# yuxiaoxiangyong/Multilateral-Temporal-view-Pyramid-Transformer-for-Video-Inpainting-Detection

Hardware: AMD Instinct MI355X
Metric: clips/sec fwd (B=8,T=5,224x224) (higher is better)
Workload: dtype f32; 1 GPU; full Mumpy forward (3 temporal views, pyramid decoder), B=8 clips/GPU, T=5, 224x224, fp32, tubelets (5,4,1); global_batch=8, launch=hipGraph replay, fork/join over HIP streams (independent branches co-scheduled), parallelism=batch-sharded x1, one metric all-reduce

## Files before the change

multilateral-temporal-view-pyramid-transformer-for-video-inpainting-detection_amd/csrc/common.h:

```cpp
#pragma once
#include <hip/hip_runtime.h>
#include <stdint.h>
#include <stdio.h>
#include "../../include/mumpy_hip.h"

namespace mumpy {

typedef float f32x4 __attribute__((ext_vector_type(4)));
typedef float f32x16 __attribute__((ext_vector_type(16)));

constexpr int WAVE = 64;
constexpr int WS = 7;
constexpr int WT = 49;
constexpr int HD = 32;

void set_error(const char* fmt, ...);

#ifdef MUMPY_TUNING
int tune_int(const char* name, int dflt);
const char* tune_str(const char* name);
#else
inline int tune_int(const char*, int dflt) { return dflt; }
inline const char* tune_str(const char*) { return nullptr; }
#endif

inline hipStream_t as_stream(void* s) { return reinterpret_cast<hipStream_t>(s); }
inline bool aligned16(const void* p) { return (reinterpret_cast<uintptr_t>(p) & 15u) == 0; }

#define MUMPY_CHECK_LAUNCH(name)                                                     \
    do {                                                                             \
        hipError_t e_ = hipGetLastError();                                           \
        if (e_ != hipSuccess) {                                                      \
            mumpy::set_error("%s: launch failed: %s", name, hipGetErrorString(e_));  \
            return (int)e_;                                                          \
        }                                                                            \
    } while (0)

#define MUMPY_REQUIRE(cond, code, ...)                                               \
    do {                                                                             \
        if (!(cond)) {                                                               \
            mumpy::set_error(__VA_ARGS__);                                           \
            return code;                                                             \
        }                                                                            \
    } while (0)

__device__ __forceinline__ unsigned xcd_major_id(unsigned orig, unsigned nwg) {
    const unsigned xcd = orig & 7, q8 = nwg >> 3, r8 = nwg & 7;
    return (xcd < r8 ? xcd * (q8 + 1) : r8 * (q8 + 1) + (xcd - r8) * q8) + (orig >> 3);
}

template <int CTRL>
__device__ __forceinline__ float dpp_f(float v) {
    return __builtin_bit_cast(float, __builtin_amdgcn_update_dpp(0, __builtin_bit_cast(int, v), CTRL, 0xF, 0xF, true));
}
__device__ __forceinline__ float swz_xor16(float v) {
    return __builtin_bit_cast(float, __builtin_amdgcn_ds_swizzle(__builtin_bit_cast(int, v), (16 << 10) | 0x1f));
}

__device__ __forceinline__ float wave_sum(float v, int width) {
    if (width > 1) v += dpp_f<0xB1>(v);
    if (width > 2) v += dpp_f<0x4E>(v);
    if (width > 4) v += dpp_f<0x141>(v);
    if (width > 8) v += dpp_f<0x140>(v);
    if (width > 16) v += swz_xor16(v);
    if (width > 32) v += __shfl_xor(v, 32);
    return v;
}

template <typename T>
__device__ __forceinline__ T ordered_sum(T first, const T* __restrict__ p, int64_t stride, int n_more) {
    T s = first;
    int z = 0;
    for (; z + 8 <= n_more; z += 8) {
        T v[8];
#pragma unroll
        for (int u = 0; u < 8; ++u) v[u] = p[(int64_t)(z + u) * stride];
#pragma unroll
        for (int u = 0; u < 8; ++u) s += v[u];
    }
    for (; z < n_more; ++z) s += p[(int64_t)z * stride];
    return s;
}

__device__ __forceinline__ void gn_block_stats(const float* __restrict__ stats, int nsplit, int G, int b, double n, float eps,
                                               float* gm, float* gr, double (*red)[2]) {
    const int tid = threadIdx.x, nslice = 256 / G, g = tid % G, k = tid / G;
    double s = 0.0, q = 0.0;
    if (k < nslice)
        for (int sp = k; sp < nsplit; sp += nslice) {
            const float* o = stats + (((int64_t)b * nsplit + sp) * G + g) * 2;
            s += (double)o[0]; q += (double)o[1];
        }
    red[tid][0] = s; red[tid][1] = q;
    __syncthreads();
    if (tid < G) {
        double ss = 0.0, qq = 0.0;
        for (int j = 0; j < nslice; ++j) { ss += red[j * G + tid][0]; qq += red[j * G + tid][1]; }
        const double m = ss / n;
        double var = qq / n - m * m;
        if (var < 0.0) var = 0.0;
        gm[tid] = (float)m;
        gr[tid] = (float)(1.0 / sqrt(var + (double)eps));
    }
    __syncthreads();
}

__device__ __forceinline__ float erf_fast(float x) {
    const float ax = fabsf(x);
    const float t = __builtin_amdgcn_rcpf(fmaf(0.3275911f, ax, 1.0f));
    float p = fmaf(1.061405429f, t, -1.453152027f);
    p = fmaf(p, t, 1.421413741f);
    p = fmaf(p, t, -0.284496736f);
    p = fmaf(p, t, 0.254829592f);
    const float y = 1.0f - p * t * __expf(-ax * ax);
    return copysignf(y, x);
}

__device__ __forceinline__ float gelu_erf(float x) { return 0.5f * x * (1.0f + erf_fast(x * 0.70710678118654752440f)); }

__device__ __forceinline__ int window_token(int wy, int wx, int p, int Hs, int W, int shift) {
    int py = p / WS, px = p - py * WS;
    int y = wy * WS + py + shift;
    int x = wx * WS + px + shift;
    if (y >= Hs) y -= Hs;
    if (x >= W) x -= W;
    return y * W + x;
}

}
```

multilateral-temporal-view-pyramid-transformer-for-video-inpainting-detection_amd/csrc/cva_fused.hip:

```cpp
#include "common.h"
using namespace mumpy;

namespace {

constexpr int BK = 32, LDR = 36;

__device__ __forceinline__ void divmod49(unsigned m, unsigned& q, unsigned& r) {
    q = (unsigned)(((uint64_t)m * 2804876602ull) >> 37);
    r = m - 49u * q;
}

template <int C>
__global__ __launch_bounds__(256, 2) void deform_sample_kv_kernel(const float* __restrict__ x2, const float* __restrict__ pos,
                                                                  const float* __restrict__ Wkv, const float* __restrict__ bkv,
                                                                  float* __restrict__ kv, int Hs2, int W, int nWx, int nW2, int nq,
                                                                  int M, unsigned gn) {
    constexpr int BM = 64, BN = 192, TN = 3, N = 2 * C, K = C, CG = C / 3, NK = K / BK, CPG = CG / BK;
    constexpr int A_LD = BM / 32, B_LD = BN / 32;
    __shared__ __attribute__((aligned(16))) float lds[2][(BM + BN) * LDR];
    const int tid = threadIdx.x, lane = tid & 63, wave = tid >> 6;
    const int c = lane & 31, h = lane >> 5, wm = wave >> 1, wn = wave & 1;
    const unsigned wgid = xcd_major_id(blockIdx.x, gridDim.x);
    const unsigned tm = wgid / gn, tn = wgid - tm * gn;
    const int m0 = (int)tm * BM, n0 = (int)tn * BN;
    const int ld_row = tid >> 3, ld_c4 = tid & 7;

    const float* abase[A_LD];
    const float* apos[A_LD];
    int aoff[A_LD][4];
    float aw[A_LD][4];
#pragma unroll
    for (int i = 0; i < A_LD; ++i) {
        int m = m0 + ld_row + 32 * i;
        if (m > M - 1) m = M - 1;
        unsigned b2, p;
        divmod49((unsigned)m, b2, p);
        const unsigned b = b2 / (unsigned)nW2, n = b2 - b * (unsigned)nW2;
        const unsigned wy = n / (unsigned)nWx, wx = n - wy * (unsigned)nWx;
        abase[i] = x2 + (((int64_t)b * Hs2 + wy * WS) * W + wx * WS) * C + 4 * ld_c4;
        apos[i] = pos + ((int64_t)(b2 % (unsigned)nq) * 3 * WT + p) * 2;
    }
    auto set_group = [&](int g) {
#pragma unroll
        for (int i = 0; i < A_LD; ++i) {
            const float gy = apos[i][g * WT * 2], gx = apos[i][g * WT * 2 + 1];
            const float iy = ((gy + 1.0f) * 0.5f) * 6.0f;
            const float ix = ((gx + 1.0f) * 0.5f) * 6.0f;
            const float y0f = floorf(iy), x0f = floorf(ix);
            const int y0 = (int)y0f, x0 = (int)x0f;
            const float wgt[4] = {(x0f + 1.0f - ix) * (y0f + 1.0f - iy), (ix - x0f) * (y0f + 1.0f - iy),
                                  (x0f + 1.0f - ix) * (iy - y0f), (ix - x0f) * (iy - y0f)};
#pragma unroll
            for (int e = 0; e < 4; ++e) {
                const int yy = y0 + (e >> 1), xx = x0 + (e & 1);
                const bool ok = (unsigned)yy < (unsigned)WS && (unsigned)xx < (unsigned)WS;
                aw[i][e] = ok ? wgt[e] : 0.f;
                aoff[i][e] = ok ? (yy * W + xx) * C : 0;
            }
        }
    };
    const float* brow[B_LD];
#pragma unroll
    for (int i = 0; i < B_LD; ++i) {
        int n = n0 + ld_row + 32 * i;
        if (n > N - 1) n = N - 1;
        brow[i] = Wkv + (int64_t)n * K + 4 * ld_c4;
    }
    f32x4 areg[A_LD], breg[B_LD];
    auto gload = [&](int kc) {
        const int k0 = kc * BK;
#pragma unroll
        for (int i = 0; i < A_LD; ++i) {
            const float* s = abase[i] + k0;
            f32x4 r = *reinterpret_cast<const f32x4*>(s + aoff[i][0]) * aw[i][0];
            r += *reinterpret_cast<const f32x4*>(s + aoff[i][1]) * aw[i][1];
            r += *reinterpret_cast<const f32x4*>(s + aoff[i][2]) * aw[i][2];
            r += *reinterpret_cast<const f32x4*>(s + aoff[i][3]) * aw[i][3];
            areg[i] = r;
        }
#pragma unroll
        for (int i = 0; i < B_LD; ++i) breg[i] = *reinterpret_cast<const f32x4*>(brow[i] + k0);
    };
    auto lstore = [&](int buf) {
#pragma unroll
        for (int i = 0; i < A_LD; ++i) *reinterpret_cast<f32x4*>(&lds[buf][(ld_row + 32 * i) * LDR + 4 * ld_c4]) = areg[i];
#pragma unroll
        for (int i = 0; i < B_LD; ++i) *reinterpret_cast<f32x4*>(&lds[buf][(BM + ld_row + 32 * i) * LDR + 4 * ld_c4]) = breg[i];
    };
    f32x16 acc[TN];
#pragma unroll
    for (int j = 0; j < TN; ++j)
#pragma unroll
        for (int r = 0; r < 16; ++r) acc[j][r] = 0.f;
    auto compute = [&](int buf) {
        const float* a_f = &lds[buf][(wm * 32 + c) * LDR + 16 * h];
        const float* b_f = &lds[buf][(BM + wn * 96 + c) * LDR + 16 * h];
#pragma unroll
        for (int q = 0; q < 4; ++q) {
            const f32x4 fa = *reinterpret_cast<const f32x4*>(a_f + 4 * q);
            f32x4 fb[TN];
#pragma unroll
            for (int j = 0; j < TN; ++j) fb[j] = *reinterpret_cast<const f32x4*>(b_f + 32 * j * LDR + 4 * q);
#pragma unroll
            for (int e = 0; e < 4; ++e)
#pragma unroll
                for (int j = 0; j < TN; ++j) acc[j] = __builtin_amdgcn_mfma_f32_32x32x2f32(fa[e], fb[j][e], acc[j], 0, 0, 0);
        }
    };
    set_group(0);
    gload(0);
    lstore(0);
    __syncthreads();
    for (int kc = 0; kc < NK; ++kc) {
        if (kc + 1 < NK) {
            if ((kc + 1) % CPG == 0) set_group((kc + 1) / CPG);
            gload(kc + 1);
        }
        compute(kc & 1);
        if (kc + 1 < NK) lstore((kc + 1) & 1);
        __syncthreads();
    }
#pragma unroll
    for (int j = 0; j < TN; ++j) {
        const int n = n0 + wn * 96 + 32 * j + c;
        if (n >= N) continue;
        const float bv = bkv[n];
#pragma unroll
        for (int r = 0; r < 16; ++r) {
            const int m = m0 + wm * 32 + (r & 3) + 8 * (r >> 2) + 4 * h;
            if (m < M) kv[(int64_t)m * N + n] = acc[j][r] + bv;
        }
    }
}

template <int C>
__global__ __launch_bounds__(256, 2) void deform_out_combine_kernel(const float* __restrict__ o, const float* __restrict__ Wout,
                                                                   const float* __restrict__ bout, const float* __restrict__ x1,
                                                                   float* __restrict__ out, int H, int W, int nWx, int nWf, int MO,
                                                                   unsigned gn) {
    constexpr int BM = 64, BN = 64, K = C, NK = K / BK;
    constexpr int A_LD = BM / 32, B_LD = BN / 32;
    __shared__ __attribute__((aligned(16))) float lds[2][(BM + BN) * LDR];
    const int tid = threadIdx.x, lane = tid & 63, wave = tid >> 6;
    const int c = lane & 31, h = lane >> 5, wm = wave >> 1, wn = wave & 1;
    const unsigned wgid = xcd_major_id(blockIdx.x, gridDim.x);
    const unsigned tn = wgid / gn, tm = wgid - tn * gn;
    const int c0 = (int)tm * BM, m0 = (int)tn * BN;
    const int ld_row = tid >> 3, ld_c4 = tid & 7;
    const float* arow[A_LD];
    const float* brow[B_LD];
#pragma unroll
    for (int i = 0; i < A_LD; ++i) {
        int cc = c0 + ld_row + 32 * i;
        if (cc > C - 1) cc = C - 1;
        arow[i] = Wout + (int64_t)cc * K + 4 * ld_c4;
    }
#pragma unroll
    for (int i = 0; i < B_LD; ++i) {
        int m = m0 + ld_row + 32 * i;
        if (m > MO - 1) m = MO - 1;
        brow[i] = o + (int64_t)m * K + 4 * ld_c4;
    }
    f32x4 areg[A_LD], breg[B_LD];
    auto gload = [&](int kc) {
#pragma unroll
        for (int i = 0; i < A_LD; ++i) areg[i] = *reinterpret_cast<const f32x4*>(arow[i] + kc * BK);
#pragma unroll
        for (int i = 0; i < B_LD; ++i) breg[i] = *reinterpret_cast<const f32x4*>(brow[i] + kc * BK);
    };
    auto lstore = [&](int buf) {
#pragma unroll
        for (int i = 0; i < A_LD; ++i) *reinterpret_cast<f32x4*>(&lds[buf][(ld_row + 32 * i) * LDR + 4 * ld_c4]) = areg[i];
#pragma unroll
        for (int i = 0; i < B_LD; ++i) *reinterpret_cast<f32x4*>(&lds[buf][(BM + ld_row + 32 * i) * LDR + 4 * ld_c4]) = breg[i];
    };
    f32x16 acc;
#pragma unroll
    for (int r = 0; r < 16; ++r) acc[r] = 0.f;
    auto compute = [&](int buf) {
        const float* a_f = &lds[buf][(wm * 32 + c) * LDR + 16 * h];
        const float* b_f = &lds[buf][(BM + wn * 32 + c) * LDR + 16 * h];
#pragma unroll
        for (int q = 0; q < 4; ++q) {
            const f32x4 fa = *reinterpret_cast<const f32x4*>(a_f + 4 * q), fb = *reinterpret_cast<const f32x4*>(b_f + 4 * q);
#pragma unroll
            for (int e = 0; e < 4; ++e) acc = __builtin_amdgcn_mfma_f32_32x32x2f32(fa[e], fb[e], acc, 0, 0, 0);
        }
    };
    gload(0);
    lstore(0);
    __syncthreads();
    for (int kc = 0; kc < NK; ++kc) {
        if (kc + 1 < NK) gload(kc + 1);
        compute(kc & 1);
        if (kc + 1 < NK) lstore((kc + 1) & 1);
        __syncthreads();
    }
    const int m = m0 + wn * 32 + c;
    if (m >= MO) return;
    unsigned bw, pp;
    divmod49((unsigned)m, bw, pp);
    const unsigned b = bw / (unsigned)nWf, n = bw - b * (unsigned)nWf;
    const int wy = (int)(n / (unsigned)nWx), wx = (int)(n - (n / (unsigned)nWx) * (unsigned)nWx);
    const int64_t img = (int64_t)b * H * W;
    const int64_t win_base = (img + (int64_t)n * WT) * C;
#pragma unroll
    for (int r = 0; r < 16; ++r) {
        const int cc = c0 + wm * 32 + (r & 3) + 8 * (r >> 2) + 4 * h;
        if (cc >= C) continue;
        const int f = cc * WT + (int)pp;
        const int po = f / C, co = f - po * C;
        const int tok = window_token(wy, wx, po, H, W, 0);
        out[win_base + f] = x1[win_base + f] + x1[(img + tok) * C + co] + (acc[r] + bout[cc]);
    }
}

}

extern "C" int mumpy_deform_sample_kv_fwd(const float* x2, const float* pos, const float* Wkv, const float* bkv, float* kv, int B,
                                          int Hs2, int W, int C, int nq, void* stream) {
    MUMPY_REQUIRE(x2 && pos && Wkv && bkv && kv, MUMPY_ENULL, "deform_sample_kv: null pointer");
    MUMPY_REQUIRE(aligned16(x2) && aligned16(Wkv) && aligned16(kv), MUMPY_EALIGN, "deform_sample_kv: pointers must be 16-byte aligned");
    MUMPY_REQUIRE(B > 0 && Hs2 > 0 && W > 0 && Hs2 % WS == 0 && W % WS == 0 && nq > 0, MUMPY_EINVAL,
                  "deform_sample_kv: bad grid (%d,%d) / nq=%d", Hs2, W, nq);
    MUMPY_REQUIRE(C == 96 || C == 192 || C == 384 || C == 768, MUMPY_EINVAL,
                  "deform_sample_kv: C=%d is not one of the encoder widths 96/192/384/768", C);
    const int nWx = W / WS, nW2 = (Hs2 / WS) * nWx;
    const int64_t nwin = (int64_t)B * nW2, M = nwin * WT;
    MUMPY_REQUIRE(M < (1ll << 31) - 64, MUMPY_ERANGE, "deform_sample_kv: too many windows");
    const unsigned gn = (unsigned)((2 * C + 191) / 192);
    const int64_t grid = ((M + 63) / 64) * gn;
    MUMPY_REQUIRE(grid < (1ll << 31), MUMPY_ERANGE, "deform_sample_kv: too many tiles");
#define MUMPY_SKV(C_)                                                                                                     \
    hipLaunchKernelGGL(deform_sample_kv_kernel<C_>, dim3((unsigned)grid), dim3(256), 0, as_stream(stream), x2, pos, Wkv, bkv, \
                       kv, Hs2, W, nWx, nW2, nq, (int)M, gn)
    switch (C) {
        case 96: MUMPY_SKV(96); break;
        case 192: MUMPY_SKV(192); break;
        case 384: MUMPY_SKV(384); break;
        default: MUMPY_SKV(768); break;
    }
#undef MUMPY_SKV
    MUMPY_CHECK_LAUNCH("deform_sample_kv");
    return 0;
}

extern "C" int mumpy_deform_out_combine_fwd(const float* o, const float* Wout, const float* bout, const float* x1, float* out, int B,
                                            int H, int W, int C, void* stream) {
    MUMPY_REQUIRE(o && Wout && bout && x1 && out, MUMPY_ENULL, "deform_out_combine: null pointer");
    MUMPY_REQUIRE(x1 != out, MUMPY_EINVAL, "deform_out_combine: out must not alias x1");
    MUMPY_REQUIRE(aligned16(o) && aligned16(Wout), MUMPY_EALIGN, "deform_out_combine: pointers must be 16-byte aligned");
    MUMPY_REQUIRE(B > 0 && H > 0 && W > 0 && H % WS == 0 && W % WS == 0, MUMPY_EINVAL, "deform_out_combine: bad grid (%d,%d)", H, W);
    MUMPY_REQUIRE(C == 96 || C == 192 || C == 384 || C == 768, MUMPY_EINVAL,
                  "deform_out_combine: C=%d is not one of the encoder widths 96/192/384/768", C);
    const int nWx = W / WS, nWf = (H / WS) * nWx;
    const int64_t MO = (int64_t)B * nWf * WT;
    MUMPY_REQUIRE(MO * 49 < (1ll << 31) && MO < (1ll << 31) - 64, MUMPY_ERANGE, "deform_out_combine: too many windows");
    const unsigned gn = (unsigned)((C + 63) / 64);
    const int64_t grid = ((MO + 63) / 64) * gn;
#define MUMPY_OC(C_)                                                                                                      \
    hipLaunchKernelGGL(deform_out_combine_kernel<C_>, dim3((unsigned)grid), dim3(256), 0, as_stream(stream), o, Wout, bout, x1, \
                       out, H, W, nWx, nWf, (int)MO, gn)
    switch (C) {
        case 96: MUMPY_OC(96); break;
        case 192: MUMPY_OC(192); break;
        case 384: MUMPY_OC(384); break;
        default: MUMPY_OC(768); break;
    }
#undef MUMPY_OC
    MUMPY_CHECK_LAUNCH("deform_out_combine");
    return 0;
}
```

multilateral-temporal-view-pyramid-transformer-for-video-inpainting-detection_amd/csrc/deform.hip:

```cpp
#include <stdlib.h>
#include "common.h"
using namespace mumpy;

namespace {

template <int Cg>
__global__ __launch_bounds__(256) void deform_offsets_kernel(const float* __restrict__ q, const float* __restrict__ dw_w,
                                                             const float* __restrict__ dw_b,
                                                             const float* __restrict__ ln_g,
                                                             const float* __restrict__ ln_b,
                                                             const float* __restrict__ pw_w, float* __restrict__ pos,
                                                             int H, int W, int C, int nWx, int nWf) {
    constexpr int CP = Cg + 4;
    __shared__ __attribute__((aligned(16))) float sm[WT * Cg + WT * CP + 25 * Cg + 4 * Cg];
    float* tile = sm;
    float* conv = sm + WT * Cg;
    float* wsm = conv + WT * CP;
    float* par = wsm + 25 * Cg;
    const int bw = blockIdx.x, g = blockIdx.y;
    const int b = bw / nWf, n = bw - b * nWf;
    const int wy = n / nWx, wx = n - wy * nWx;
    const int tid = threadIdx.x;
    const int64_t L = (int64_t)H * W;
    const float* qb = q + (int64_t)b * L * C + g * Cg;
    const int cg4 = Cg >> 2;
    {
        constexpr int NT = WT * (Cg / 4), PT = (NT + 255) / 256;
        f32x4 v[PT];
#pragma unroll
        for (int u = 0; u < PT; ++u) {
            const int idx = tid + 256 * u;
            if (idx < NT) {
                const int p = idx / cg4, c4 = idx - p * cg4;
                v[u] = *reinterpret_cast<const f32x4*>(qb + (int64_t)window_token(wy, wx, p, H, W, 0) * C + 4 * c4);
            }
        }
#pragma unroll
        for (int u = 0; u < PT; ++u) {
            const int idx = tid + 256 * u;
            if (idx < NT) { const int p = idx / cg4, c4 = idx - p * cg4; *reinterpret_cast<f32x4*>(tile + p * Cg + 4 * c4) = v[u]; }
        }
        constexpr int NW = 25 * Cg / 4, PW = (NW + 255) / 256;
        f32x4 t[PW];
#pragma unroll
        for (int u = 0; u < PW; ++u) { const int idx = tid + 256 * u; if (idx < NW) t[u] = reinterpret_cast<const f32x4*>(dw_w)[idx]; }
#pragma unroll
        for (int u = 0; u < PW; ++u) { const int idx = tid + 256 * u; if (idx < NW) reinterpret_cast<f32x4*>(wsm)[idx] = t[u]; }
    }
    for (int idx = tid; idx < Cg; idx += 256) {
        par[idx] = ln_g[idx];
        par[Cg + idx] = ln_b[idx];
        par[2 * Cg + idx] = pw_w[idx];
        par[3 * Cg + idx] = pw_w[Cg + idx];
    }
    const int cc = tid % Cg;
    const float breg = dw_b[cc];
    __syncthreads();
    float wreg[25];
#pragma unroll
    for (int i = 0; i < 25; ++i) wreg[i] = wsm[cc * 25 + i];
    for (int p = tid / Cg; p < WT; p += 256 / Cg) {
        const int py = p / WS, px = p - py * WS;
        float acc = breg;
#pragma unroll
        for (int dy = 0; dy < 5; ++dy) {
            const int yy = py + dy - 2;
            const bool vy = (unsigned)yy < (unsigned)WS;
            const int yc = vy ? yy : py;
#pragma unroll
            for (int dx = 0; dx < 5; ++dx) {
                const int xx = px + dx - 2;
                const bool ok = vy && (unsigned)xx < (unsigned)WS;
                const int xc = ok ? xx : px;
                const float t = tile[(yc * WS + xc) * Cg + cc];
                acc = fmaf(ok ? t : 0.f, wreg[dy * 5 + dx], acc);
            }
        }
        conv[p * CP + cc] = acc;
    }
    __syncthreads();
    const int p = tid >> 2, qd = tid & 3;
    if (p < WT) {
        const float* cv = conv + p * CP;
        float s = 0.f;
#pragma unroll 8
        for (int ch = qd; ch < Cg; ch += 4) s += cv[ch];
        s += __shfl_xor(s, 1);
        s += __shfl_xor(s, 2);
        const float mean = s / (float)Cg;
        float qq = 0.f;
#pragma unroll 8
        for (int ch = qd; ch < Cg; ch += 4) { const float d = cv[ch] - mean; qq = fmaf(d, d, qq); }
        qq += __shfl_xor(qq, 1);
        qq += __shfl_xor(qq, 2);
        const float rstd = rsqrtf(qq / (float)Cg + 1e-5f);
        float oy = 0.f, ox = 0.f;
#pragma unroll 4
        for (int ch = qd; ch < Cg; ch += 4) {
            const float a = gelu_erf((cv[ch] - mean) * rstd * par[ch] + par[Cg + ch]);
            oy = fmaf(a, par[2 * Cg + ch], oy);
            ox = fmaf(a, par[3 * Cg + ch], ox);
        }
        oy += __shfl_xor(oy, 1);
        oy += __shfl_xor(oy, 2);
        ox += __shfl_xor(ox, 1);
        ox += __shfl_xor(ox, 2);
        if (qd == 0) {
            const int py = p / WS, px = p - py * WS;
            const float ry = ((0.5f + (float)py) / 7.0f) * 2.0f - 1.0f;
            const float rx = ((0.5f + (float)px) / 7.0f) * 2.0f - 1.0f;
            const float rng = 1.0f / 7.0f;
            float* o = pos + (((int64_t)bw * 3 + g) * WT + p) * 2;
            o[0] = tanhf(oy) * rng * 2.0f + ry;
            o[1] = tanhf(ox) * rng * 2.0f + rx;
        }
    }
}

template <int C>
__global__ __launch_bounds__(256) void deform_sample_kernel(const float* __restrict__ x2, const float* __restrict__ pos,
                                                            float* __restrict__ out, int Hs2, int W, int nWx, int nW2,
                                                            int nq) {
    constexpr int C4N = C / 4, CG = C / 3;
    const int b2 = blockIdx.x;
    const int b = b2 / nW2, n = b2 - b * nW2;
    const int wy = n / nWx, wx = n - wy * nWx;
    const float* base = x2 + ((int64_t)b * Hs2 * W + (int64_t)wy * WS * W + wx * WS) * C;
    const float* pw = pos + (int64_t)(b2 % nq) * 3 * WT * 2;
    float* ob = out + (int64_t)b2 * WT * C;
    for (int idx = threadIdx.x; idx < WT * C4N; idx += 256) {
        const int p = idx / C4N, c4 = idx - p * C4N;
        const int g = (4 * c4) / CG;
        const float gy = pw[(g * WT + p) * 2], gx = pw[(g * WT + p) * 2 + 1];
        const float iy = ((gy + 1.0f) * 0.5f) * 6.0f;
        const float ix = ((gx + 1.0f) * 0.5f) * 6.0f;
        const float y0f = floorf(iy), x0f = floorf(ix);
        const int y0 = (int)y0f, x0 = (int)x0f;
        const float wnw = (x0f + 1.0f - ix) * (y0f + 1.0f - iy);
        const float wne = (ix - x0f) * (y0f + 1.0f - iy);
        const float wsw = (x0f + 1.0f - ix) * (iy - y0f);
        const float wse = (ix - x0f) * (iy - y0f);
        const float* src = base + 4 * c4;
        auto corner = [&](int yy, int xx) -> f32x4 {
            if (yy < 0 || yy >= WS || xx < 0 || xx >= WS) return f32x4{0, 0, 0, 0};
            return *reinterpret_cast<const f32x4*>(src + (yy * W + xx) * C);
        };
        f32x4 r = corner(y0, x0) * wnw;
        r += corner(y0, x0 + 1) * wne;
        r += corner(y0 + 1, x0) * wsw;
        r += corner(y0 + 1, x0 + 1) * wse;
        *reinterpret_cast<f32x4*>(ob + idx * 4) = r;
    }
}

template <int C>
__global__ __launch_bounds__(256) void deform_sample_lds_kernel(const float* __restrict__ x2, const float* __restrict__ pos,
                                                                float* __restrict__ out, int Hs2, int W, int nWx, int nW2,
                                                                int nq) {
    constexpr int SL = 96, S4 = SL / 4, CG = C / 3;
    __shared__ __attribute__((aligned(16))) float tile[WT * SL];
    const int b2 = blockIdx.x, slab = blockIdx.y;
    const int b = b2 / nW2, n = b2 - b * nW2;
    const int wy = n / nWx, wx = n - wy * nWx;
    const float* base = x2 + ((int64_t)b * Hs2 * W + (int64_t)wy * WS * W + wx * WS) * C + slab * SL;
    for (int idx = threadIdx.x; idx < WT * S4; idx += 256) {
        const int tok = idx / S4, j = idx - tok * S4;
        const int ty = tok / WS, tx = tok - ty * WS;
        *reinterpret_cast<f32x4*>(&tile[tok * SL + 4 * j]) = *reinterpret_cast<const f32x4*>(base + (ty * W + tx) * C + 4 * j);
    }
    __syncthreads();
    const float* pw = pos + (int64_t)(b2 % nq) * 3 * WT * 2;
    float* ob = out + (int64_t)b2 * WT * C + slab * SL;
    for (int idx = threadIdx.x; idx < WT * S4; idx += 256) {
        const int p = idx / S4, c4 = idx - p * S4;
        const int g = (slab * SL + 4 * c4) / CG;
        const float gy = pw[(g * WT + p) * 2], gx = pw[(g * WT + p) * 2 + 1];
        const float iy = ((gy + 1.0f) * 0.5f) * 6.0f;
        const float ix = ((gx + 1.0f) * 0.5f) * 6.0f;
        const float y0f = floorf(iy), x0f = floorf(ix);
        const int y0 = (int)y0f, x0 = (int)x0f;
        const float wnw = (x0f + 1.0f - ix) * (y0f + 1.0f - iy);
        const float wne = (ix - x0f) * (y0f + 1.0f - iy);
        const float wsw = (x0f + 1.0f - ix) * (iy - y0f);
        const float wse = (ix - x0f) * (iy - y0f);
        auto corner = [&](int yy, int xx) -> f32x4 {
            if (yy < 0 || yy >= WS || xx < 0 || xx >= WS) return f32x4{0, 0, 0, 0};
            return *reinterpret_cast<const f32x4*>(&tile[(yy * WS + xx) * SL + 4 * c4]);
        };
        f32x4 r = corner(y0, x0) * wnw;
        r += corner(y0, x0 + 1) * wne;
        r += corner(y0 + 1, x0) * wsw;
        r += corner(y0 + 1, x0 + 1) * wse;
        *reinterpret_cast<f32x4*>(ob + p * C + 4 * c4) = r;
    }
}

__global__ __launch_bounds__(256) void deform_combine_kernel(const float* __restrict__ x1, const float* __restrict__ Yt,
                                                             float* __restrict__ out, int H, int W, int C, int nWx,
                                                             int nWf) {
    __shared__ float tile[WT * 33];
    const int bw = blockIdx.x, cb = blockIdx.y;
    const int b = bw / nWf, n = bw - b * nWf;
    const int wy = n / nWx, wx = n - wy * nWx;
    const int tid = threadIdx.x;
    const float* ys = Yt + (int64_t)bw * WT * C + cb * 32;
    for (int idx = tid; idx < WT * 32; idx += 256) {
        const int p = idx >> 5, cc = idx & 31;
        tile[p * 33 + cc] = ys[(int64_t)p * C + cc];
    }
    __syncthreads();
    const int64_t img = (int64_t)b * H * W;
    const int64_t win_base = (img + (int64_t)n * WT) * C;
    const int f0 = cb * 32 * WT;
    for (int idx = tid; idx < WT * 32; idx += 256) {
        const int f = f0 + idx;
        const int cl = idx / WT, pp = idx - cl * WT;
        const int po = f / C, co = f - po * C;
        const int tok = window_token(wy, wx, po, H, W, 0);
        out[win_base + f] = x1[win_base + f] + x1[(img + tok) * C + co] + tile[pp * 33 + cl];
    }
}

__global__ __launch_bounds__(256) void add_kernel(const float* __restrict__ a, const float* __restrict__ b,
                                                  float* __restrict__ o, int64_t n4) {
    for (int64_t i = (int64_t)blockIdx.x * 256 + threadIdx.x; i < n4; i += (int64_t)gridDim.x * 256)
        reinterpret_cast<f32x4*>(o)[i] = reinterpret_cast<const f32x4*>(a)[i] + reinterpret_cast<const f32x4*>(b)[i];
}

}

extern "C" int mumpy_deform_offsets_fwd(const float* q, const float* dw_w, const float* dw_b, const float* ln_g,
                                        const float* ln_b, const float* pw_w, float* pos, int B, int H, int W, int C,
                                        void* stream) {
    MUMPY_REQUIRE(q && dw_w && dw_b && ln_g && ln_b && pw_w && pos, MUMPY_ENULL, "deform_offsets: null pointer");
    MUMPY_REQUIRE(aligned16(q) && aligned16(dw_w), MUMPY_EALIGN, "deform_offsets: q and the depthwise weights must be 16-byte aligned");
    MUMPY_REQUIRE(B > 0 && H % WS == 0 && W % WS == 0 && H > 0 && W > 0, MUMPY_EINVAL, "deform_offsets: bad grid (%d,%d)", H, W);
    const int Cg = C / 3;
    MUMPY_REQUIRE(C % 3 == 0 && (Cg == 32 || Cg == 64 || Cg == 128 || Cg == 256), MUMPY_EINVAL,
                  "deform_offsets: group width C/3=%d must be 32, 64, 128 or 256", Cg);
    const int nWx = W / WS, nWf = (H / WS) * nWx;
#define MUMPY_OFFS(CG)                                                                                              \
    hipLaunchKernelGGL(deform_offsets_kernel<CG>, dim3(B * nWf, 3), dim3(256), 0, as_stream(stream), q, dw_w, dw_b, ln_g, \
                       ln_b, pw_w, pos, H, W, C, nWx, nWf)
    switch (Cg) {
        case 32: MUMPY_OFFS(32); break;
        case 64: MUMPY_OFFS(64); break;
        case 128: MUMPY_OFFS(128); break;
        default: MUMPY_OFFS(256); break;
    }
#undef MUMPY_OFFS
    MUMPY_CHECK_LAUNCH("deform_offsets");
    return 0;
}

extern "C" int mumpy_deform_sample_fwd(const float* x2, const float* pos, float* out, int B, int Hs2, int W, int C,
                                       int nq, void* stream) {
    MUMPY_REQUIRE(x2 && pos && out, MUMPY_ENULL, "deform_sample: null pointer");
    MUMPY_REQUIRE(aligned16(x2) && aligned16(out), MUMPY_EALIGN, "deform_sample: pointers must be 16-byte aligned");
    MUMPY_REQUIRE(B > 0 && Hs2 > 0 && W > 0 && Hs2 % WS == 0 && W % WS == 0 && nq > 0, MUMPY_EINVAL,
                  "deform_sample: bad grid (%d,%d) / nq=%d", Hs2, W, nq);
    MUMPY_REQUIRE(C == 96 || C == 192 || C == 384 || C == 768, MUMPY_EINVAL,
                  "deform_sample: C=%d is not one of the encoder widths 96/192/384/768", C);
    const int nWx = W / WS, nW2 = (Hs2 / WS) * nWx;
    const int64_t nwin = (int64_t)B * nW2;
    MUMPY_REQUIRE(nwin < (1ll << 31), MUMPY_ERANGE, "deform_sample: too many windows");
    static const bool direct = tune_int("MUMPY_SAMPLE_DIRECT", 0) != 0;
#define MUMPY_SAMPLE(C_)                                                                                             \
    if (direct)                                                                                                      \
        hipLaunchKernelGGL(deform_sample_kernel<C_>, dim3((unsigned)nwin), dim3(256), 0, as_stream(stream), x2, pos, out,  \
                           Hs2, W, nWx, nW2, nq);                                                                    \
    else                                                                                                             \
        hipLaunchKernelGGL(deform_sample_lds_kernel<C_>, dim3((unsigned)nwin, C_ / 96), dim3(256), 0, as_stream(stream), x2, \
                           pos, out, Hs2, W, nWx, nW2, nq)
    switch (C) {
        case 96: MUMPY_SAMPLE(96); break;
        case 192: MUMPY_SAMPLE(192); break;
        case 384: MUMPY_SAMPLE(384); break;
        default: MUMPY_SAMPLE(768); break;
    }
#undef MUMPY_SAMPLE
    MUMPY_CHECK_LAUNCH("deform_sample");
    return 0;
}

extern "C" int mumpy_deform_combine_fwd(const float* x1, const float* Yt, float* out, int B, int H, int W, int C,
                                        void* stream) {
    MUMPY_REQUIRE(x1 && Yt && out, MUMPY_ENULL, "deform_combine: null pointer");
    MUMPY_REQUIRE(x1 != out, MUMPY_EINVAL, "deform_combine: out must not alias x1");
    MUMPY_REQUIRE(B > 0 && H > 0 && W > 0 && H % WS == 0 && W % WS == 0 && C % 32 == 0, MUMPY_EINVAL,
                  "deform_combine: bad shape (%d,%d,%d)", H, W, C);
    const int nWx = W / WS, nWf = (H / WS) * nWx;
    hipLaunchKernelGGL(deform_combine_kernel, dim3(B * nWf, C / 32), dim3(256), 0, as_stream(stream), x1, Yt, out, H, W,
                       C, nWx, nWf);
    MUMPY_CHECK_LAUNCH("deform_combine");
    return 0;
}

extern "C" int mumpy_add_fwd(const float* a, const float* b, float* out, int64_t n, void* stream) {
    MUMPY_REQUIRE(a && b && out, MUMPY_ENULL, "add: null pointer");
    MUMPY_REQUIRE(aligned16(a) && aligned16(b) && aligned16(out) && n % 4 == 0 && n >= 0, MUMPY_EALIGN,
                  "add: need 16-byte aligned pointers and n %% 4 == 0");
    if (n == 0) return 0;
    int64_t grid = (n / 4 + 255) / 256;
    if (grid > 4096) grid = 4096;
    hipLaunchKernelGGL(add_kernel, dim3((unsigned)grid), dim3(256), 0, as_stream(stream), a, b, out, n / 4);
    MUMPY_CHECK_LAUNCH("add");
    return 0;
}
```

Baseline: 375.1 clips/s.

## Specialize deform kernels for small grids with deeper prefetch and row-split offsets

```diff
diff --git a/multilateral-temporal-view-pyramid-transformer-for-video-inpainting-detection_amd/csrc/common.h b/multilateral-temporal-view-pyramid-transformer-for-video-inpainting-detection_amd/csrc/common.h
--- a/multilateral-temporal-view-pyramid-transformer-for-video-inpainting-detection_amd/csrc/common.h
+++ b/multilateral-temporal-view-pyramid-transformer-for-video-inpainting-detection_amd/csrc/common.h
@@ -13,6 +13,7 @@
 constexpr int WS = 7;
 constexpr int WT = 49;
 constexpr int HD = 32;
+constexpr int CHIP_CUS = 256;
 
 void set_error(const char* fmt, ...);
 
diff --git a/multilateral-temporal-view-pyramid-transformer-for-video-inpainting-detection_amd/csrc/cva_fused.hip b/multilateral-temporal-view-pyramid-transformer-for-video-inpainting-detection_amd/csrc/cva_fused.hip
--- a/multilateral-temporal-view-pyramid-transformer-for-video-inpainting-detection_amd/csrc/cva_fused.hip
+++ b/multilateral-temporal-view-pyramid-transformer-for-video-inpainting-detection_amd/csrc/cva_fused.hip
@@ -10,7 +10,7 @@
     r = m - 49u * q;
 }
 
-template <int C>
+template <int C, bool AHEAD>
 __global__ __launch_bounds__(256, 2) void deform_sample_kv_kernel(const float* __restrict__ x2, const float* __restrict__ pos,
                                                                   const float* __restrict__ Wkv, const float* __restrict__ bkv,
                                                                   float* __restrict__ kv, int Hs2, int W, int nWx, int nW2, int nq,
@@ -26,7 +26,7 @@
     const int ld_row = tid >> 3, ld_c4 = tid & 7;
 
     const float* abase[A_LD];
-    const float* apos[A_LD];
+    float gpy[A_LD][3], gpx[A_LD][3];
     int aoff[A_LD][4];
     float aw[A_LD][4];
 #pragma unroll
@@ -38,12 +38,19 @@
         const unsigned b = b2 / (unsigned)nW2, n = b2 - b * (unsigned)nW2;
         const unsigned wy = n / (unsigned)nWx, wx = n - wy * (unsigned)nWx;
         abase[i] = x2 + (((int64_t)b * Hs2 + wy * WS) * W + wx * WS) * C + 4 * ld_c4;
-        apos[i] = pos + ((int64_t)(b2 % (unsigned)nq) * 3 * WT + p) * 2;
+        const float* ap = pos + ((int64_t)(b2 % (unsigned)nq) * 3 * WT + p) * 2;
+#pragma unroll
+        for (int g = 0; g < 3; ++g) {
+            const float2 gp = *reinterpret_cast<const float2*>(ap + g * WT * 2);
+            gpy[i][g] = gp.x;
+            gpx[i][g] = gp.y;
+        }
     }
     auto set_group = [&](int g) {
 #pragma unroll
         for (int i = 0; i < A_LD; ++i) {
-            const float gy = apos[i][g * WT * 2], gx = apos[i][g * WT * 2 + 1];
+            const float gy = g == 0 ? gpy[i][0] : g == 1 ? gpy[i][1] : gpy[i][2];
+            const float gx = g == 0 ? gpx[i][0] : g == 1 ? gpx[i][1] : gpx[i][2];
             const float iy = ((gy + 1.0f) * 0.5f) * 6.0f;
             const float ix = ((gx + 1.0f) * 0.5f) * 6.0f;
             const float y0f = floorf(iy), x0f = floorf(ix);
@@ -66,24 +73,32 @@
         if (n > N - 1) n = N - 1;
         brow[i] = Wkv + (int64_t)n * K + 4 * ld_c4;
     }
-    f32x4 areg[A_LD], breg[B_LD];
+    f32x4 araw[A_LD][4], areg[A_LD], breg[B_LD];
+    auto blend = [&](int i) {
+        f32x4 r = araw[i][0] * aw[i][0];
+        r += araw[i][1] * aw[i][1];
+        r += araw[i][2] * aw[i][2];
+        r += araw[i][3] * aw[i][3];
+        return r;
+    };
     auto gload = [&](int kc) {
         const int k0 = kc * BK;
 #pragma unroll
         for (int i = 0; i < A_LD; ++i) {
             const float* s = abase[i] + k0;
-            f32x4 r = *reinterpret_cast<const f32x4*>(s + aoff[i][0]) * aw[i][0];
-            r += *reinterpret_cast<const f32x4*>(s + aoff[i][1]) * aw[i][1];
-            r += *reinterpret_cast<const f32x4*>(s + aoff[i][2]) * aw[i][2];
-            r += *reinterpret_cast<const f32x4*>(s + aoff[i][3]) * aw[i][3];
-            areg[i] = r;
+#pragma unroll
+            for (int e = 0; e < 4; ++e) araw[i][e] = *reinterpret_cast<const f32x4*>(s + aoff[i][e]);
+            if constexpr (!AHEAD) areg[i] = blend(i);
         }
 #pragma unroll
         for (int i = 0; i < B_LD; ++i) breg[i] = *reinterpret_cast<const f32x4*>(brow[i] + k0);
     };
     auto lstore = [&](int buf) {
 #pragma unroll
-        for (int i = 0; i < A_LD; ++i) *reinterpret_cast<f32x4*>(&lds[buf][(ld_row + 32 * i) * LDR + 4 * ld_c4]) = areg[i];
+        for (int i = 0; i < A_LD; ++i) {
+            if constexpr (AHEAD) areg[i] = blend(i);
+            *reinterpret_cast<f32x4*>(&lds[buf][(ld_row + 32 * i) * LDR + 4 * ld_c4]) = areg[i];
+        }
 #pragma unroll
         for (int i = 0; i < B_LD; ++i) *reinterpret_cast<f32x4*>(&lds[buf][(BM + ld_row + 32 * i) * LDR + 4 * ld_c4]) = breg[i];
     };
@@ -116,7 +131,9 @@
             if ((kc + 1) % CPG == 0) set_group((kc + 1) / CPG);
             gload(kc + 1);
         }
+        if constexpr (AHEAD) __builtin_amdgcn_sched_barrier(0);
         compute(kc & 1);
+        if constexpr (AHEAD) __builtin_amdgcn_sched_barrier(0);
         if (kc + 1 < NK) lstore((kc + 1) & 1);
         __syncthreads();
     }
@@ -133,14 +150,15 @@
     }
 }
 
-template <int C>
-__global__ __launch_bounds__(256, 2) void deform_out_combine_kernel(const float* __restrict__ o, const float* __restrict__ Wout,
+template <int C, int PF>
+__global__ __launch_bounds__(256, PF > 2 ? 1 : 2) void deform_out_combine_kernel(const float* __restrict__ o, const float* __restrict__ Wout,
                                                                    const float* __restrict__ bout, const float* __restrict__ x1,
                                                                    float* __restrict__ out, int H, int W, int nWx, int nWf, int MO,
                                                                    unsigned gn) {
-    constexpr int BM = 64, BN = 64, K = C, NK = K / BK;
+    constexpr int BM = 64, BN = 64, K = C, NK = K / BK, NS = NK / PF;
     constexpr int A_LD = BM / 32, B_LD = BN / 32;
-    __shared__ __attribute__((aligned(16))) float lds[2][(BM + BN) * LDR];
+    static_assert(NK % PF == 0, "a step is PF whole chunks");
+    __shared__ __attribute__((aligned(16))) float lds[2 * PF][(BM + BN) * LDR];
     const int tid = threadIdx.x, lane = tid & 63, wave = tid >> 6;
     const int c = lane & 31, h = lane >> 5, wm = wave >> 1, wn = wave & 1;
     const unsigned wgid = xcd_major_id(blockIdx.x, gridDim.x);
@@ -161,18 +179,25 @@
         if (m > MO - 1) m = MO - 1;
         brow[i] = o + (int64_t)m * K + 4 * ld_c4;
     }
-    f32x4 areg[A_LD], breg[B_LD];
-    auto gload = [&](int kc) {
-#pragma unroll
-        for (int i = 0; i < A_LD; ++i) areg[i] = *reinterpret_cast<const f32x4*>(arow[i] + kc * BK);
-#pragma unroll
-        for (int i = 0; i < B_LD; ++i) breg[i] = *reinterpret_cast<const f32x4*>(brow[i] + kc * BK);
-    };
-    auto lstore = [&](int buf) {
-#pragma unroll
-        for (int i = 0; i < A_LD; ++i) *reinterpret_cast<f32x4*>(&lds[buf][(ld_row + 32 * i) * LDR + 4 * ld_c4]) = areg[i];
-#pragma unroll
-        for (int i = 0; i < B_LD; ++i) *reinterpret_cast<f32x4*>(&lds[buf][(BM + ld_row + 32 * i) * LDR + 4 * ld_c4]) = breg[i];
+    f32x4 areg[PF][A_LD], breg[PF][B_LD];
+    auto gload = [&](int st) {
+#pragma unroll
+        for (int j = 0; j < PF; ++j) {
+#pragma unroll
+            for (int i = 0; i < A_LD; ++i) areg[j][i] = *reinterpret_cast<const f32x4*>(arow[i] + (st * PF + j) * BK);
+#pragma unroll
+            for (int i = 0; i < B_LD; ++i) breg[j][i] = *reinterpret_cast<const f32x4*>(brow[i] + (st * PF + j) * BK);
+        }
+    };
+    auto lstore = [&](int set) {
+#pragma unroll
+        for (int j = 0; j < PF; ++j) {
+            float* d = lds[set * PF + j];
+#pragma unroll
+            for (int i = 0; i < A_LD; ++i) *reinterpret_cast<f32x4*>(&d[(ld_row + 32 * i) * LDR + 4 * ld_c4]) = areg[j][i];
+#pragma unroll
+            for (int i = 0; i < B_LD; ++i) *reinterpret_cast<f32x4*>(&d[(BM + ld_row + 32 * i) * LDR + 4 * ld_c4]) = breg[j][i];
+        }
     };
     f32x16 acc;
 #pragma unroll
@@ -190,10 +215,13 @@
     gload(0);
     lstore(0);
     __syncthreads();
-    for (int kc = 0; kc < NK; ++kc) {
-        if (kc + 1 < NK) gload(kc + 1);
-        compute(kc & 1);
-        if (kc + 1 < NK) lstore((kc + 1) & 1);
+    for (int st = 0; st < NS; ++st) {
+        if (st + 1 < NS) gload(st + 1);
+        if constexpr (PF > 1) __builtin_amdgcn_sched_barrier(0);
+#pragma unroll
+        for (int j = 0; j < PF; ++j) compute((st & 1) * PF + j);
+        if constexpr (PF > 1) __builtin_amdgcn_sched_barrier(0);
+        if (st + 1 < NS) lstore((st + 1) & 1);
         __syncthreads();
     }
     const int m = m0 + wn * 32 + c;
@@ -231,15 +259,18 @@
     const unsigned gn = (unsigned)((2 * C + 191) / 192);
     const int64_t grid = ((M + 63) / 64) * gn;
     MUMPY_REQUIRE(grid < (1ll << 31), MUMPY_ERANGE, "deform_sample_kv: too many tiles");
-#define MUMPY_SKV(C_)                                                                                                     \
-    hipLaunchKernelGGL(deform_sample_kv_kernel<C_>, dim3((unsigned)grid), dim3(256), 0, as_stream(stream), x2, pos, Wkv, bkv, \
-                       kv, Hs2, W, nWx, nW2, nq, (int)M, gn)
+    const bool ahead = grid <= CHIP_CUS;
+#define MUMPY_SKV(C_, AH_)                                                                                                \
+    hipLaunchKernelGGL((deform_sample_kv_kernel<C_, AH_>), dim3((unsigned)grid), dim3(256), 0, as_stream(stream), x2, pos, Wkv, \
+                       bkv, kv, Hs2, W, nWx, nW2, nq, (int)M, gn)
+#define MUMPY_SKV2(C_) if (ahead) MUMPY_SKV(C_, true); else MUMPY_SKV(C_, false)
     switch (C) {
-        case 96: MUMPY_SKV(96); break;
-        case 192: MUMPY_SKV(192); break;
-        case 384: MUMPY_SKV(384); break;
-        default: MUMPY_SKV(768); break;
-    }
+        case 96: MUMPY_SKV2(96); break;
+        case 192: MUMPY_SKV2(192); break;
+        case 384: MUMPY_SKV2(384); break;
+        default: MUMPY_SKV2(768); break;
+    }
+#undef MUMPY_SKV2
 #undef MUMPY_SKV
     MUMPY_CHECK_LAUNCH("deform_sample_kv");
     return 0;
@@ -258,14 +289,15 @@
     MUMPY_REQUIRE(MO * 49 < (1ll << 31) && MO < (1ll << 31) - 64, MUMPY_ERANGE, "deform_out_combine: too many windows");
     const unsigned gn = (unsigned)((C + 63) / 64);
     const int64_t grid = ((MO + 63) / 64) * gn;
-#define MUMPY_OC(C_)                                                                                                      \
-    hipLaunchKernelGGL(deform_out_combine_kernel<C_>, dim3((unsigned)grid), dim3(256), 0, as_stream(stream), o, Wout, bout, x1, \
-                       out, H, W, nWx, nWf, (int)MO, gn)
+    const bool deep = grid <= CHIP_CUS;
+#define MUMPY_OC(C_, PF_)                                                                                                 \
+    hipLaunchKernelGGL((deform_out_combine_kernel<C_, PF_>), dim3((unsigned)grid), dim3(256), 0, as_stream(stream), o, Wout, bout, \
+                       x1, out, H, W, nWx, nWf, (int)MO, gn)
     switch (C) {
-        case 96: MUMPY_OC(96); break;
-        case 192: MUMPY_OC(192); break;
-        case 384: MUMPY_OC(384); break;
-        default: MUMPY_OC(768); break;
+        case 96: MUMPY_OC(96, 1); break;
+        case 192: MUMPY_OC(192, 1); break;
+        case 384: if (deep) MUMPY_OC(384, 4); else MUMPY_OC(384, 1); break;
+        default: if (deep) MUMPY_OC(768, 4); else MUMPY_OC(768, 1); break;
     }
 #undef MUMPY_OC
     MUMPY_CHECK_LAUNCH("deform_out_combine");
diff --git a/multilateral-temporal-view-pyramid-transformer-for-video-inpainting-detection_amd/csrc/deform.hip b/multilateral-temporal-view-pyramid-transformer-for-video-inpainting-detection_amd/csrc/deform.hip
--- a/multilateral-temporal-view-pyramid-transformer-for-video-inpainting-detection_amd/csrc/deform.hip
+++ b/multilateral-temporal-view-pyramid-transformer-for-video-inpainting-detection_amd/csrc/deform.hip
@@ -4,20 +4,25 @@
 
 namespace {
 
-template <int Cg>
+template <int Cg, int RB>
 __global__ __launch_bounds__(256) void deform_offsets_kernel(const float* __restrict__ q, const float* __restrict__ dw_w,
                                                              const float* __restrict__ dw_b,
                                                              const float* __restrict__ ln_g,
                                                              const float* __restrict__ ln_b,
                                                              const float* __restrict__ pw_w, float* __restrict__ pos,
                                                              int H, int W, int C, int nWx, int nWf) {
+    static_assert(RB == WS || RB == 1, "a block takes the whole window or one row of it");
     constexpr int CP = Cg + 4;
-    __shared__ __attribute__((aligned(16))) float sm[WT * Cg + WT * CP + 25 * Cg + 4 * Cg];
+    constexpr int HALO = RB == WS ? 0 : 2;
+    constexpr int TR = RB + 2 * HALO, NP = RB * WS;
+    __shared__ __attribute__((aligned(16))) float sm[TR * WS * Cg + NP * CP + 25 * Cg + 4 * Cg];
     float* tile = sm;
-    float* conv = sm + WT * Cg;
-    float* wsm = conv + WT * CP;
+    float* conv = sm + TR * WS * Cg;
+    float* wsm = conv + NP * CP;
     float* par = wsm + 25 * Cg;
     const int bw = blockIdx.x, g = blockIdx.y;
+    const int r0 = RB == WS ? 0 : (int)blockIdx.z * RB;
+    const int ro = r0 - HALO;
     const int b = bw / nWf, n = bw - b * nWf;
     const int wy = n / nWx, wx = n - wy * nWx;
     const int tid = threadIdx.x;
@@ -25,20 +30,22 @@
     const float* qb = q + (int64_t)b * L * C + g * Cg;
     const int cg4 = Cg >> 2;
     {
-        constexpr int NT = WT * (Cg / 4), PT = (NT + 255) / 256;
+        constexpr int NT = TR * WS * (Cg / 4), PT = (NT + 255) / 256;
         f32x4 v[PT];
 #pragma unroll
         for (int u = 0; u < PT; ++u) {
             const int idx = tid + 256 * u;
-            if (idx < NT) {
-                const int p = idx / cg4, c4 = idx - p * cg4;
+            const int lp = idx / cg4, c4 = idx - lp * cg4;
+            const int p = lp + ro * WS;
+            if (idx < NT && (unsigned)p < (unsigned)WT)
                 v[u] = *reinterpret_cast<const f32x4*>(qb + (int64_t)window_token(wy, wx, p, H, W, 0) * C + 4 * c4);
-            }
         }
 #pragma unroll
         for (int u = 0; u < PT; ++u) {
             const int idx = tid + 256 * u;
-            if (idx < NT) { const int p = idx / cg4, c4 = idx - p * cg4; *reinterpret_cast<f32x4*>(tile + p * Cg + 4 * c4) = v[u]; }
+            const int lp = idx / cg4, c4 = idx - lp * cg4;
+            const int p = lp + ro * WS;
+            if (idx < NT && (unsigned)p < (unsigned)WT) *reinterpret_cast<f32x4*>(tile + lp * Cg + 4 * c4) = v[u];
         }
         constexpr int NW = 25 * Cg / 4, PW = (NW + 255) / 256;
         f32x4 t[PW];
@@ -59,8 +66,9 @@
     float wreg[25];
 #pragma unroll
     for (int i = 0; i < 25; ++i) wreg[i] = wsm[cc * 25 + i];
-    for (int p = tid / Cg; p < WT; p += 256 / Cg) {
-        const int py = p / WS, px = p - py * WS;
+    for (int pl = tid / Cg; pl < NP; pl += 256 / Cg) {
+        const int ly = pl / WS, px = pl - ly * WS;
+        const int py = r0 + ly;
         float acc = breg;
 #pragma unroll
         for (int dy = 0; dy < 5; ++dy) {
@@ -72,16 +80,16 @@
                 const int xx = px + dx - 2;
                 const bool ok = vy && (unsigned)xx < (unsigned)WS;
                 const int xc = ok ? xx : px;
-                const float t = tile[(yc * WS + xc) * Cg + cc];
+                const float t = tile[((yc - ro) * WS + xc) * Cg + cc];
                 acc = fmaf(ok ? t : 0.f, wreg[dy * 5 + dx], acc);
             }
         }
-        conv[p * CP + cc] = acc;
+        conv[pl * CP + cc] = acc;
     }
     __syncthreads();
-    const int p = tid >> 2, qd = tid & 3;
-    if (p < WT) {
-        const float* cv = conv + p * CP;
+    const int pl = tid >> 2, qd = tid & 3;
+    if (pl < NP) {
+        const float* cv = conv + pl * CP;
         float s = 0.f;
 #pragma unroll 8
         for (int ch = qd; ch < Cg; ch += 4) s += cv[ch];
@@ -106,6 +114,7 @@
         ox += __shfl_xor(ox, 1);
         ox += __shfl_xor(ox, 2);
         if (qd == 0) {
+            const int p = r0 * WS + pl;
             const int py = p / WS, px = p - py * WS;
             const float ry = ((0.5f + (float)py) / 7.0f) * 2.0f - 1.0f;
             const float rx = ((0.5f + (float)px) / 7.0f) * 2.0f - 1.0f;
@@ -239,9 +248,15 @@
     MUMPY_REQUIRE(C % 3 == 0 && (Cg == 32 || Cg == 64 || Cg == 128 || Cg == 256), MUMPY_EINVAL,
                   "deform_offsets: group width C/3=%d must be 32, 64, 128 or 256", Cg);
     const int nWx = W / WS, nWf = (H / WS) * nWx;
+    static const int force_rows = tune_int("MUMPY_OFFSETS_ROWS", -1);
+    const bool rows = force_rows >= 0 ? force_rows != 0 : (int64_t)B * nWf * 3 < CHIP_CUS;
 #define MUMPY_OFFS(CG)                                                                                              \
-    hipLaunchKernelGGL(deform_offsets_kernel<CG>, dim3(B * nWf, 3), dim3(256), 0, as_stream(stream), q, dw_w, dw_b, ln_g, \
-                       ln_b, pw_w, pos, H, W, C, nWx, nWf)
+    if (rows)                                                                                                       \
+        hipLaunchKernelGGL((deform_offsets_kernel<CG, 1>), dim3(B * nWf, 3, WS), dim3(256), 0, as_stream(stream), q, dw_w, dw_b, \
+                           ln_g, ln_b, pw_w, pos, H, W, C, nWx, nWf);                                               \
+    else                                                                                                            \
+        hipLaunchKernelGGL((deform_offsets_kernel<CG, WS>), dim3(B * nWf, 3), dim3(256), 0, as_stream(stream), q, dw_w, dw_b, \
+                           ln_g, ln_b, pw_w, pos, H, W, C, nWx, nWf)
     switch (Cg) {
         case 32: MUMPY_OFFS(32); break;
         case 64: MUMPY_OFFS(64); break;
```

Result: no change. 376.3 clips/s (median of 4 runs) (+0.3%).
